# AlexeyAB/yolo2_light

Measured on NVIDIA H100. Metric: images/sec, higher is better.
Workload: dtype bf16

## Files before the change

### yolo2_light_b200/csrc/yb_conv_tc.cu

```cuda
#include <cuda.h>
#include <cuda_bf16.h>
#include <cuda_runtime.h>

#include <algorithm>
#include <climits>
#include <cstdlib>
#include <cstring>
#include <memory>
#include <string>
#include <type_traits>
#include <vector>

#include "yb_conv_tc.cuh"
#include "yb_cuda.h"

namespace yb {

namespace {

constexpr int TC_BM = 128;
constexpr int TC_EPI_WARPS = 8;
constexpr int TC_THREADS = 32 * TC_EPI_WARPS + 32;
constexpr int TC_PRODUCER_WARP = TC_EPI_WARPS;
constexpr int TC_ACC_BAR = 3;
// ... 9 lines not shown
    uint32_t acc;
};

struct TcParams {
    int N;
    int TW, TWlog2, TH;
    int xt, jt, nt;
    int num_work;
    int kind;
    int kk;
    float alpha1;
    const float *mean;
    int xK;
    int *acc_out;
    float *yolo_out;
    int yolo_per;
    int PR, row_off;
    int OH, OW, OHp, OWp;
    int size, cblocks, kblocks;
    int BK, BN;
    int stride2;
    int xoff, yoff;
    int stages;
    uint32_t stage_bytes, a_bytes, b_bytes;
    int bstat;
    uint32_t bstat_bytes;
    int tma_epi;
    uint32_t stg_bytes;
    int acc_pitch;
    int pool_fmt, jshift;
    float pool_mult;
    signed char *pool_out; long pool_ldc; int pool_Hp, pool_Wp;
    int sps;
    TcSmem sm;
    uint32_t desc_hi;
    char *out; long out_ldc; int n;
    const char *res;
    const float *bias; int act, act2;
    unsigned long long *stats;
    int dbg;
};

__device__ __forceinline__ uint32_t smem_u32(const void *p) { return (uint32_t)__cvta_generic_to_shared(p); }

__device__ __forceinline__ bool elect_one() {
    uint32_t pred = 0;
    asm volatile(
        "{\n\t.reg .b32 rx;\n\t.reg .pred px;\n\telect.sync rx|px, %1;\n\t@px mov.s32 %0, 1;\n\t}"
        : "+r"(pred) : "r"(0xffffffffu));
    return pred != 0;
}

__device__ __forceinline__ void mbar_init(uint32_t bar, uint32_t count) {
    asm volatile("mbarrier.init.shared::cta.b64 [%0], %1;" ::"r"(bar), "r"(count));
}
__device__ __forceinline__ void mbar_arrive_expect_tx(uint32_t bar, uint32_t bytes) {
    asm volatile("mbarrier.arrive.expect_tx.shared::cta.b64 _, [%0], %1;" ::"r"(bar), "r"(bytes) : "memory");
}
__device__ __forceinline__ void mbar_arrive(uint32_t bar) {
    asm volatile("mbarrier.arrive.shared::cta.b64 _, [%0];" ::"r"(bar) : "memory");
}
__device__ __forceinline__ uint32_t mbar_try_wait(uint32_t bar, uint32_t parity) {
    uint32_t ok;
    asm volatile(
        "{\n\t.reg .pred p;\n\tmbarrier.try_wait.parity.shared::cta.b64 p, [%1], %2;\n\tselp.b32 %0, 1, 0, p;\n\t}"
        : "=r"(ok) : "r"(bar), "r"(parity) : "memory");
    return ok;
}
__device__ __forceinline__ void mbar_wait(uint32_t bar, uint32_t parity) {
    if (mbar_try_wait(bar, parity)) return;
    const long long t0 = clock64();
    while (!mbar_try_wait(bar, parity))
        if (clock64() - t0 > 4000000000LL) __trap();
}

__device__ __forceinline__ void tma_load_3d(uint32_t dst, const CUtensorMap *tm, uint32_t bar, int c0, int c1, int c2) {
    asm volatile(
        "cp.async.bulk.tensor.3d.shared::cluster.global.tile.mbarrier::complete_tx::bytes [%0], [%1, {%3, %4, %5}], [%2];"
        ::"r"(dst), "l"(tm), "r"(bar), "r"(c0), "r"(c1), "r"(c2) : "memory");
}
__device__ __forceinline__ uint64_t l2_policy_evict_first() {
    uint64_t pol;
    asm volatile("createpolicy.fractional.L2::evict_first.b64 %0, 1.0;" : "=l"(pol));
    return pol;
}
__device__ __forceinline__ void tma_load_3d_hint(uint32_t dst, const CUtensorMap *tm, uint32_t bar, int c0, int c1, int c2, uint64_t pol) {
    asm volatile(
        "cp.async.bulk.tensor.3d.shared::cluster.global.tile.mbarrier::complete_tx::bytes.L2::cache_hint [%0], [%1, {%3, %4, %5}], [%2], %6;"
        ::"r"(dst), "l"(tm), "r"(bar), "r"(c0), "r"(c1), "r"(c2), "l"(pol) : "memory");
}
__device__ __forceinline__ void tma_load_2d(uint32_t dst, const CUtensorMap *tm, uint32_t bar, int c0, int c1) {
    asm volatile(
        "cp.async.bulk.tensor.2d.shared::cluster.global.tile.mbarrier::complete_tx::bytes [%0], [%1, {%3, %4}], [%2];"
        ::"r"(dst), "l"(tm), "r"(bar), "r"(c0), "r"(c1) : "memory");
}
__device__ __forceinline__ void tma_load_5d(uint32_t dst, const CUtensorMap *tm, uint32_t bar, int c0, int c1, int c2,
                                            int c3, int c4) {
    asm volatile(
        "cp.async.bulk.tensor.5d.shared::cluster.global.tile.mbarrier::complete_tx::bytes [%0], [%1, {%3, %4, %5, %6, %7}], [%2];"
        ::"r"(dst), "l"(tm), "r"(bar), "r"(c0), "r"(c1), "r"(c2), "r"(c3), "r"(c4) : "memory");
}

__device__ __forceinline__ void tma_store_3d(const CUtensorMap *tm, uint32_t src, int c0, int c1, int c2) {
    asm volatile("cp.async.bulk.tensor.3d.global.shared::cta.bulk_group [%0, {%2, %3, %4}], [%1];"
                 ::"l"(tm), "r"(src), "r"(c0), "r"(c1), "r"(c2) : "memory");
}
__device__ __forceinline__ void tma_store_commit() { asm volatile("cp.async.bulk.commit_group;" ::: "memory"); }
__device__ __forceinline__ void tma_store_wait_read0() { asm volatile("cp.async.bulk.wait_group.read 0;" ::: "memory"); }
__device__ __forceinline__ void tma_store_wait_all() { asm volatile("cp.async.bulk.wait_group 0;" ::: "memory"); }
__device__ __forceinline__ void named_bar_sync(int id, int nthreads) {
    asm volatile("bar.sync %0, %1;" ::"r"(id), "r"(nthreads) : "memory");
}
__device__ __forceinline__ void prefetch_tmap(const CUtensorMap *tm) { asm volatile("prefetch.tensormap [%0];" ::"l"(tm) : "memory"); }
__device__ __forceinline__ void fence_mbar_init() { asm volatile("fence.mbarrier_init.release.cluster;" ::: "memory"); }
__device__ __forceinline__ void pdl_wait_and_launch() {
    asm volatile("griddepcontrol.wait;" ::: "memory");
    asm volatile("griddepcontrol.launch_dependents;" ::: "memory");
}

__device__ __forceinline__ uint64_t wg_desc(uint32_t addr, uint32_t hi) {
    return ((uint64_t)hi << 32) | (uint64_t)(((addr & 0x3FFFFu) >> 4) | (1u << 16));
}
__device__ __forceinline__ void wg_fence() { asm volatile("wgmma.fence.sync.aligned;" ::: "memory"); }
__device__ __forceinline__ void wg_commit() { asm volatile("wgmma.commit_group.sync.aligned;" ::: "memory"); }
template <int N>
__device__ __forceinline__ void wg_wait() { asm volatile("wgmma.wait_group.sync.aligned %0;" ::"n"(N) : "memory"); }
template <typename T, int N>
// ... 108 lines not shown
};

__device__ __forceinline__ uint32_t pack_bf16x2(float a, float b) {
    __nv_bfloat162 h = __floats2bfloat162_rn(a, b);
    return *reinterpret_cast<uint32_t *>(&h);
}

__device__ __forceinline__ void acc_ld32(uint32_t addr, uint32_t (&v)[32]) {
#pragma unroll
    for (int c = 0; c < 8; ++c)
        asm volatile("ld.shared.v4.b32 {%0, %1, %2, %3}, [%4];" : "=r"(v[4 * c]), "=r"(v[4 * c + 1]), "=r"(v[4 * c + 2]), "=r"(v[4 * c + 3])
                     : "r"(addr + 16u * (uint32_t)c) : "memory");
}
template <typename T, int NR>
__device__ __forceinline__ void acc_store_frag(uint32_t acc, int pitch, int row0, const T (&d)[NR]) {
    const int lane = threadIdx.x & 31, w = (threadIdx.x >> 5) & 3;
    const int r = row0 + 16 * w + (lane >> 2), c = 2 * (lane & 3);
    const uint32_t a0 = acc + 4u * (uint32_t)(r * pitch + c), a1 = a0 + 4u * 8u * (uint32_t)pitch;
#pragma unroll
    for (int j = 0; j < NR / 4; ++j) {
        asm volatile("st.shared.v2.b32 [%0], {%1, %2};" ::"r"(a0 + 32u * (uint32_t)j), "r"(*reinterpret_cast<const uint32_t *>(&d[4 * j])),
                     "r"(*reinterpret_cast<const uint32_t *>(&d[4 * j + 1])) : "memory");
        asm volatile("st.shared.v2.b32 [%0], {%1, %2};" ::"r"(a1 + 32u * (uint32_t)j), "r"(*reinterpret_cast<const uint32_t *>(&d[4 * j + 2])),
                     "r"(*reinterpret_cast<const uint32_t *>(&d[4 * j + 3])) : "memory");
    }
}

__device__ __forceinline__ uint32_t smem_base(const void *smem_raw) { return (smem_u32(smem_raw) + 1023u) & ~1023u; }
__device__ __forceinline__ void *smem_ptr(uint32_t addr) { return __cvta_shared_to_generic(addr); }
__device__ __forceinline__ void st_shared_u32(uint32_t addr, uint32_t v) {
    asm volatile("st.shared.b32 [%0], %1;" ::"r"(addr), "r"(v) : "memory");
}

struct TcItem { int n0, x0, J0; };
__device__ __forceinline__ TcItem tc_item(const TcParams &p, int w, int BN) {
    const int m = w / p.nt;
    return {(w % p.nt) * BN, (m % p.xt) * p.TW, (m / p.xt) * p.TH + p.jshift};
}
struct TcPixel {
    int img, oy, ox;
    __device__ __forceinline__ bool valid(const TcParams &p) const { return img < p.N && oy >= 0 && oy < p.OH && ox < p.OW; }
};
__device__ __forceinline__ TcPixel tc_pixel(const TcParams &p, const TcItem &t, int r) {
    const int J = t.J0 + (r >> p.TWlog2);
    const int img = J / p.PR;
    return {img, J - img * p.PR - p.row_off, t.x0 + (r & (p.TW - 1))};
}

struct TcRing {
    int stage = 0;
    uint32_t phase = 0;
    __device__ __forceinline__ void advance(int stages) { if (++stage == stages) { stage = 0; phase ^= 1u; } }
};
__device__ __forceinline__ void tc_init_ring(const TcParams &p, uint32_t base) {
    for (int s = 0; s < p.stages; ++s) { mbar_init(base + p.sm.full + 8u * s, 1); mbar_init(base + p.sm.empty + 8u * s, TC_EPI_WARPS); }
    mbar_init(base + p.sm.bstat_bar, 1);
}

template <int BN_MAX, typename F>
__device__ __forceinline__ void tc_dispatch(const TcParams &p, F &&f) {
    auto by_kk = [&](auto bn_c) {
        if (p.kk == 4) f(bn_c, std::integral_constant<int, 4>{});
        else if (p.kk == 2) f(bn_c, std::integral_constant<int, 2>{});
        else f(bn_c, std::integral_constant<int, 1>{});
    };
    if constexpr (BN_MAX == 256) {
        if (p.BN == 256) { by_kk(std::integral_constant<int, 256>{}); return; }
    }
    if (p.BN == 128) by_kk(std::integral_constant<int, 128>{});
    else if (p.BN == 64) by_kk(std::integral_constant<int, 64>{});
    else by_kk(std::integral_constant<int, 32>{});
}

enum TcStat {
    STAT_PROD_WAIT_EMPTY,
    STAT_PROD_TMA_ISSUE,
    STAT_PROD_TOTAL,
    STAT_CONS_WAIT_FULL,
    STAT_CONS_WAIT_READY,
    STAT_CONS_FIRST_READY,
    STAT_CONS_TOTAL,
    STAT_STORE_WAIT_FULL,
    STAT_STORE_WAIT_READ,
    TC_NSTATS = 16
};
__device__ __forceinline__ unsigned long long &tc_stat(const TcParams &p, TcStat s) { return p.stats[blockIdx.x * TC_NSTATS + s]; }
template <bool ST, typename F>
__device__ __forceinline__ void timed(long long &cycles, F &&f) {
    if constexpr (ST) { const long long c0 = clock64(); f(); cycles += clock64() - c0; }
    else f();
}

template <bool ST>
__device__ __forceinline__ void tc_produce(const CUtensorMap *tmA, const CUtensorMap *tmB, const TcParams &p, uint32_t base,
                                           int w_first, int w_step) {
    TcRing ring;
    long long w_empty = 0, w_tma = 0; const long long t_begin = ST ? clock64() : 0;
    const int sps = p.sps, kblocks = p.kblocks, cblocks = p.cblocks, BK = p.BK, fsize = p.size, stages = p.stages;
    const int xoff = p.xoff, yoff = p.yoff, stride2 = p.stride2;
    const uint32_t a_bytes = p.a_bytes, b_bytes = p.b_bytes, stage_bytes = p.stage_bytes;
    const uint32_t b_off = (uint32_t)sps * a_bytes;
    const uint32_t smemB = base, smem0 = base + p.sm.ring, bstat_bar = base + p.sm.bstat_bar;
    const int bstat = p.bstat;
    if (bstat) {
        mbar_arrive_expect_tx(bstat_bar, p.bstat_bytes);
        for (int kb = 0; kb < kblocks; ++kb) tma_load_2d(smemB + (uint32_t)kb * b_bytes, tmB, bstat_bar, kb * BK, 0);
    }
    for (int w = w_first; w < p.num_work; w += w_step) {
        const TcItem it = tc_item(p, w, p.BN);
        int cb = 0, ky = 0, kx = 0, kcol = 0;
        for (int kb0 = 0; kb0 < kblocks; kb0 += sps) {
            const int nsub = min(sps, kblocks - kb0);
            timed<ST>(w_empty, [&] { mbar_wait(base + p.sm.empty + 8u * (uint32_t)ring.stage, ring.phase ^ 1u); });
            const uint32_t fb = base + p.sm.full + 8u * (uint32_t)ring.stage;
            const uint32_t a_dst = smem0 + (uint32_t)ring.stage * stage_bytes;
            const uint32_t b_dst = a_dst + b_off;
            if (p.dbg & 1) {
                mbar_arrive(fb);
                ring.advance(stages);
                continue;
            }
            mbar_arrive_expect_tx(fb, (uint32_t)nsub * (a_bytes + (bstat ? 0u : b_bytes)));
            timed<ST>(w_tma, [&] {
                for (int j = 0; j < nsub; ++j) {
                    const uint32_t ad = a_dst + (uint32_t)j * a_bytes, bd = b_dst + (uint32_t)j * b_bytes;
                    const int c0 = cb * BK;
                    if (stride2) tma_load_5d(ad, tmA, fb, c0, kx & 1, it.x0 + (kx >> 1), ky & 1, it.J0 + (ky >> 1));
                    else tma_load_3d(ad, tmA, fb, c0, it.x0 + kx + xoff, it.J0 + ky + yoff);
                    if (!bstat) tma_load_2d(bd, tmB, fb, kcol, it.n0);
                    kcol += BK;
                    if (++cb == cblocks) { cb = 0; if (++kx == fsize) { kx = 0; ++ky; } }
                }
            });
            ring.advance(stages);
        }
    }
    if (ST && p.stats) {
        tc_stat(p, STAT_PROD_WAIT_EMPTY) = w_empty; tc_stat(p, STAT_PROD_TMA_ISSUE) = w_tma;
        tc_stat(p, STAT_PROD_TOTAL) = clock64() - t_begin;
    }
}

template <TcKind KIND, int BN, int KK, bool ST, typename T>
__device__ __forceinline__ void tc_mma_loop(T (&d)[BN / 2], const TcParams &p, uint32_t base, int wg, int lane, TcRing &ring,
                                            long long &w_full) {
#pragma unroll
    for (int i = 0; i < BN / 2; ++i) d[i] = T(0);
    wg_fence_operand(d);
    const int sps = p.sps, stages = p.stages, kblocks = p.kblocks;
    const uint32_t a_bytes = p.a_bytes, b_bytes = p.b_bytes, stage_bytes = p.stage_bytes, hi = p.desc_hi;
    const uint32_t b_off = (uint32_t)sps * a_bytes, a_wg = (uint32_t)wg * (a_bytes >> 1);
    const uint32_t smemB = base, smem0 = base + p.sm.ring;
    const uint32_t full = base + p.sm.full, empty = base + p.sm.empty;
    auto release = [&](int s) { __syncwarp(); if (lane == 0) mbar_arrive(empty + 8u * (uint32_t)s); };
    int pend = -1, jj = 0;
    for (int kb = 0; kb < kblocks; ++kb) {
        if (jj == 0) timed<ST>(w_full, [&] { mbar_wait(full + 8u * (uint32_t)ring.stage, ring.phase); });
        const uint32_t st_base = smem0 + (uint32_t)ring.stage * stage_bytes;
        const uint32_t a_kb = st_base + a_wg + (uint32_t)jj * a_bytes;
        const uint32_t b_kb = p.bstat ? smemB + (uint32_t)kb * b_bytes : st_base + b_off + (uint32_t)jj * b_bytes;
        wg_fence();
#pragma unroll
        for (int k = 0; k < KK; ++k)
            Wg<KIND, BN>::mma(d, wg_desc(a_kb + 32u * (uint32_t)k, hi), wg_desc(b_kb + 32u * (uint32_t)k, hi),
                              (kb > 0 || k > 0) ? 1u : 0u);
        wg_commit();
        wg_wait<1>();
        if (pend >= 0) { release(pend); pend = -1; }
        if (++jj == sps || kb + 1 == kblocks) {
            pend = ring.stage; jj = 0;
            ring.advance(stages);
        }
    }
    wg_wait<0>();
    wg_fence_operand(d);
    if (pend >= 0) release(pend);
}

template <Arith A>
__device__ __forceinline__ float int_epilogue(const TcParams &p, int acc, int f, float bias) {
    return IntEpi<A>::finish(acc, IntEpi<A>::MEAN ? ((f < p.n) ? __ldg(p.mean + f) : 0.f) : p.alpha1, bias, p.act);
}

template <bool ST, int EPI>
__global__ void __launch_bounds__(TC_THREADS, 1)
k_conv_tc(const __grid_constant__ CUtensorMap tmA, const __grid_constant__ CUtensorMap tmB, const __grid_constant__ CUtensorMap tmO,
          const __grid_constant__ CUtensorMap tmO1, const __grid_constant__ CUtensorMap tmR, const TcParams p) {
    extern __shared__ uint8_t smem_raw[];
    const uint32_t base = smem_base(smem_raw);

    const int warp = __shfl_sync(0xffffffffu, (int)(threadIdx.x >> 5), 0);
    const int lane = threadIdx.x & 31;
    const int w_first = (int)blockIdx.x, w_step = (int)gridDim.x;

    if (warp == TC_PRODUCER_WARP && elect_one()) {
        prefetch_tmap(&tmA);
        prefetch_tmap(&tmB);
        tc_init_ring(p, base);
        if (p.tma_epi) prefetch_tmap(&tmO);
        fence_mbar_init();
    }
    const float *bias_s = reinterpret_cast<const float *>(smem_ptr(base + p.sm.bias));
    const uint32_t *ymask_s = reinterpret_cast<const uint32_t *>(smem_ptr(base + p.sm.ymask));
    const uint32_t stg_base = base + p.sm.stg;
    const uint32_t acc_base = base + p.sm.acc;
    for (int i = threadIdx.x; i < p.nt * p.BN; i += TC_THREADS)
        st_shared_u32(base + p.sm.bias + 4u * (uint32_t)i, __float_as_uint((i < p.n) ? __ldg(p.bias + i) : 0.f));
    if (p.yolo_out) {
        for (int wd = threadIdx.x; wd < p.nt * p.BN / 32; wd += TC_THREADS) {
            uint32_t m = 0;
            for (int j = 0; j < 32; ++j) { const int e = (wd * 32 + j) % p.yolo_per; if (e == 2 || e == 3) m |= 1u << j; }
            st_shared_u32(base + p.sm.ymask + 4u * (uint32_t)wd, m);
        }
    }
    __syncthreads();
    pdl_wait_and_launch();

    if (warp == TC_PRODUCER_WARP) {
        if (elect_one()) tc_produce<ST>(&tmA, &tmB, p, base, w_first, w_step);
    } else {
        const int ew = warp;
        const int wg = ew >> 2;
        TcRing ring;
        long long w_full = 0;
        if (p.bstat) mbar_wait(base + p.sm.bstat_bar, 0);
        auto mainloop = [&](auto kind_c) {
            tc_dispatch<128>(p, [&](auto bn_c, auto kk_c) {
                constexpr TcKind KIND = decltype(kind_c)::value;
                constexpr int BN = decltype(bn_c)::value;
                constexpr int KK = decltype(kk_c)::value;
                using T = typename std::conditional<KIND == TC_S8, uint32_t, float>::type;
                T d[BN / 2];
                tc_mma_loop<KIND, BN, KK, ST>(d, p, base, wg, lane, ring, w_full);
                named_bar_sync(TC_ACC_BAR, 32 * TC_EPI_WARPS);
                acc_store_frag(acc_base, p.acc_pitch, wg * 64, d);
                named_bar_sync(TC_ACC_BAR, 32 * TC_EPI_WARPS);
            });
        };
        auto run_mainloop = [&]() {
            if constexpr (EPI == 2) mainloop(std::integral_constant<TcKind, TC_S8>{});
            else if (p.kind == TC_BF16) mainloop(std::integral_constant<TcKind, TC_BF16>{});
            else mainloop(std::integral_constant<TcKind, TC_TF32>{});
        };

        const int q = ew & 3;
        const int half = ew >> 2;
        const int cbeg = (p.BN >= 64) ? half * (p.BN >> 1) : 0;
        const int cend = (p.BN >= 64) ? cbeg + (p.BN >> 1) : (half == 0 ? p.BN : 0);
        const int r = q * 32 + lane;
        const bool leaky = p.act == ACT_LEAKY;
        const uint32_t taddr = acc_base + 4u * (uint32_t)(r * p.acc_pitch);
        const long long t_begin = ST ? clock64() : 0;
// ... 157 lines not shown
                if (p.kind == TC_XNOR) int_slabs(std::integral_constant<Arith, AR_XNOR>{});
                else if (p.kind == TC_S8_GPU) int_slabs(std::integral_constant<Arith, AR_INT8_GPU>{});
                else if (p.kind == TC_XNOR_GPU) int_slabs(std::integral_constant<Arith, AR_XNOR_GPU>{});
                else if (p.kind == TC_PM1Z_GPU) int_slabs(std::integral_constant<Arith, AR_PM1Z_GPU>{});
                else int_slabs(std::integral_constant<Arith, AR_INT8>{});
            } else {
                for (int f0 = cbeg; f0 < cend; f0 += 64) {
                    if (cend - f0 >= 64) {
                        uint32_t v0[32], v1[32];
                        acc_ld32(taddr + 4u * (uint32_t)f0, v0);
                        acc_ld32(taddr + 4u * (uint32_t)f0 + 128u, v1);
                        finish_f32(v0, f0);
                        finish_f32(v1, f0 + 32);
                    } else {
                        uint32_t v0[32];
                        acc_ld32(taddr + 4u * (uint32_t)f0, v0);
                        finish_f32(v0, f0);
                    }
                }
            }
        }
        if (EPI == 2 && p.tma_epi && q == 0 && lane == 0) tma_store_wait_all();
        if (ST && p.stats && ew == 0 && lane == 0) { tc_stat(p, STAT_CONS_WAIT_FULL) = w_full; tc_stat(p, STAT_CONS_TOTAL) = clock64() - t_begin; }
    }
}

constexpr int TCR_THREADS = 384;
constexpr int TCR_PRODUCER_REGS = 40, TCR_CONSUMER_REGS = 216;
constexpr int TCR_STORE_WARP = 9;
constexpr int TCR_MAX_SLABS = 4;

template <bool ST>
__device__ __forceinline__ void tcr_store(const CUtensorMap *tmO, const CUtensorMap *tmO1, const CUtensorMap *tmR, const TcParams &p,
                                          uint32_t buf, uint32_t stg_full, uint32_t stg_ready, int g, int w_first, int w_step) {
    const int SW = p.tma_epi, BN = p.BN;
    const uint32_t tile = 64u * 2u * (uint32_t)SW;
    const int hx = (p.TW == 128) ? 64 * g : 0, hy = (p.TW == 128) ? 0 : g * (p.TH >> 1);
    long long w_full = 0, w_read = 0;
    auto item = [&](int w, int &n0, int &x, int &y) {
        const TcItem it = tc_item(p, w, BN);
        n0 = it.n0; x = it.x0 + 1 + hx; y = it.J0 + hy;
        if (p.stride2) {
            const int i0 = y / p.PR, i1 = min((y + max(p.TH >> 1, 1) - 1) / p.PR, p.N - 1);
            y = i0 == i1 ? y + i0 + 1 : -1 - y;
        }
        return (min(BN, p.n - n0) + SW - 1) / SW;
    };
    auto store_slab = [&](uint32_t src, int c, int x, int y) {
        if (y >= 0) { tma_store_3d(tmO, src, c, x, y); return; }
        const int J0 = -1 - y;
        int img = J0 / p.PR, oy = J0 - img * p.PR;
        for (int t = 0; t < (p.TH >> 1); ++t) {
            if (img < p.N && oy < p.OH) tma_store_3d(tmO1, src, c, x, J0 + t + img + 1);
            if (++oy == p.PR) { oy = 0; ++img; }
            src += (uint32_t)(p.TW * 2 * SW);
        }
    };
    auto wait_read = [&]() { timed<ST>(w_read, tma_store_wait_read0); };
    auto load_res = [&](int s, int n0, int x, int y) {
        tma_load_3d_hint(buf + (uint32_t)s * tile, tmR, stg_ready, n0 + s * SW, x, y, l2_policy_evict_first());
    };
    if (w_first < p.num_work) {
        if (p.res) {
            int n0, x, y;
            const int ns = item(w_first, n0, x, y);
            mbar_arrive_expect_tx(stg_ready, (uint32_t)ns * tile);
            for (int s = 0; s < ns; ++s) load_res(s, n0, x, y);
        } else mbar_arrive(stg_ready);
    }
    uint32_t phases = 0;
    for (int w = w_first; w < p.num_work; w += w_step) {
        int n0, x, y, n0n = 0, xn = 0, yn = 0;
        const int ns = item(w, n0, x, y);
        const bool next = w + w_step < p.num_work, res_next = next && p.res;
        const int nsn = next ? item(w + w_step, n0n, xn, yn) : 0;
        for (int s = 0; s < ns; ++s) {
            const uint32_t fb = stg_full + 8u * (uint32_t)s;
            timed<ST>(w_full, [&] { mbar_wait(fb, (phases >> s) & 1u); });
            phases ^= 1u << s;
            if (s == 0 && res_next) mbar_arrive_expect_tx(stg_ready, (uint32_t)nsn * tile);
            store_slab(buf + (uint32_t)s * tile, n0 + s * SW, x, y);
            tma_store_commit();
            if (res_next && s < nsn) { wait_read(); load_res(s, n0n, xn, yn); }
        }
        if (res_next) {
            for (int s = ns; s < nsn; ++s) { wait_read(); load_res(s, n0n, xn, yn); }
        } else if (next) {
            wait_read();
            mbar_arrive(stg_ready);
        }
    }
    tma_store_wait_all();
    if (ST && p.stats && g == 0) { tc_stat(p, STAT_STORE_WAIT_FULL) = w_full; tc_stat(p, STAT_STORE_WAIT_READ) = w_read; }
}

template <bool ST>
__global__ void __launch_bounds__(TCR_THREADS, 1)
k_conv_tc_reg(const __grid_constant__ CUtensorMap tmA, const __grid_constant__ CUtensorMap tmB, const __grid_constant__ CUtensorMap tmO,
              const __grid_constant__ CUtensorMap tmO1, const __grid_constant__ CUtensorMap tmR, const TcParams p) {
    extern __shared__ uint8_t smem_raw[];
    const uint32_t base = smem_base(smem_raw);
    auto stg_full = [&](int g, int s) { return base + p.sm.stg_full + 8u * (uint32_t)(g * TCR_MAX_SLABS + s); };
    auto stg_ready = [&](int g) { return base + p.sm.stg_ready + 8u * (uint32_t)g; };
    float *bias_s = reinterpret_cast<float *>(smem_ptr(base + p.sm.bias));
    const uint32_t stg_base = base + p.sm.stg;

    const int warp = __shfl_sync(0xffffffffu, (int)(threadIdx.x >> 5), 0);
    const int lane = threadIdx.x & 31;
    const int wg = warp >> 2;
    const int w_first = (int)blockIdx.x, w_step = (int)gridDim.x;
    const bool epi_mem = !(p.dbg & 4);

    if (warp == TC_PRODUCER_WARP && elect_one()) {
        prefetch_tmap(&tmA);
        prefetch_tmap(&tmB);
        prefetch_tmap(&tmO);
        if (p.stride2) prefetch_tmap(&tmO1);
        if (p.res) prefetch_tmap(&tmR);
        tc_init_ring(p, base);
        for (int g = 0; g < 2; ++g) {
            for (int s = 0; s < TCR_MAX_SLABS; ++s) mbar_init(stg_full(g, s), 4);
            mbar_init(stg_ready(g), 1);
        }
        fence_mbar_init();
    }
    for (int i = threadIdx.x; i < p.nt * p.BN; i += TCR_THREADS) bias_s[i] = (i < p.n) ? __ldg(p.bias + i) : 0.f;
    __syncthreads();
    pdl_wait_and_launch();

    if (wg == 2) {
        asm volatile("setmaxnreg.dec.sync.aligned.u32 %0;" ::"n"(TCR_PRODUCER_REGS));
        if (warp == TC_PRODUCER_WARP) {
            if (elect_one()) tc_produce<ST>(&tmA, &tmB, p, base, w_first, w_step);
        } else if (warp < TCR_STORE_WARP + 2 && epi_mem) {
            const int g = warp - TCR_STORE_WARP;
            if (elect_one()) tcr_store<ST>(&tmO, &tmO1, &tmR, p, stg_base + (uint32_t)g * 128u * (uint32_t)p.BN, stg_full(g, 0), stg_ready(g), g, w_first, w_step);
        }
        return;
    }
    asm volatile("setmaxnreg.inc.sync.aligned.u32 %0;" ::"n"(TCR_CONSUMER_REGS));

    const int rl = 16 * (warp & 3) + (lane >> 2), cq = 2 * (lane & 3);
    const bool leaky = p.act == ACT_LEAKY, leaky2 = p.act2 == ACT_LEAKY;
    const bool has_res = p.res != nullptr;
    TcRing ring;
    uint32_t stg_phase = 0;
    long long w_full = 0, w_ready = 0; const long long t_begin = ST ? clock64() : 0;
    if (p.bstat) mbar_wait(base + p.sm.bstat_bar, 0);

    tc_dispatch<256>(p, [&](auto bn_c, auto kk_c) {
        constexpr int BN = decltype(bn_c)::value;
        constexpr int KK = decltype(kk_c)::value;
        constexpr int SW = BN >= 64 ? 64 : 32;
        constexpr uint32_t ROWB = SW * 2, TILE = 64u * ROWB;
        const uint32_t buf = stg_base + (uint32_t)wg * (uint32_t)(BN / SW) * TILE;
        auto slab_off = [&](int row, int c) -> uint32_t {
            const int sw = (SW == 64) ? (row & 7) : ((row >> 1) & 3);
            return (uint32_t)row * ROWB + ((uint32_t)(c ^ sw) << 4) + 2u * (uint32_t)cq;
        };
        for (int w = w_first; w < p.num_work; w += w_step) {
            float d[BN / 2];
            tc_mma_loop<TC_BF16, BN, KK, ST>(d, p, base, wg, lane, ring, w_full);
            if (!epi_mem) continue;
            const TcItem it = tc_item(p, w, BN);
            const int n0 = it.n0;
            bool valid[2];
#pragma unroll
            for (int h = 0; h < 2; ++h)
                valid[h] = tc_pixel(p, it, 64 * wg + rl + 8 * h).valid(p);
            const int nslab = (min(BN, p.n - n0) + SW - 1) / SW;
            long long dt = 0;
            timed<ST>(dt, [&] { mbar_wait(stg_ready(wg), stg_phase); });
            if (w != w_first) w_ready += dt;
            else if (ST && p.stats && warp == 0 && lane == 0) tc_stat(p, STAT_CONS_FIRST_READY) = dt;
            stg_phase ^= 1u;
#pragma unroll
            for (int s = 0; s < BN / SW; ++s) {
                if (s >= nslab) break;
                const uint32_t slab = buf + (uint32_t)s * TILE;
#pragma unroll
                for (int jj = 0; jj < SW / 8; ++jj) {
                    const int j = s * (SW / 8) + jj;
                    const float2 b = *reinterpret_cast<const float2 *>(bias_s + n0 + 8 * j + cq);
#pragma unroll
                    for (int e = 0; e < 4; ++e) {
                        const float a = d[4 * j + e] + ((e & 1) ? b.y : b.x);
                        d[4 * j + e] = leaky ? fmaxf(a, 0.1f * a) : a;
                    }
                }
                if (has_res) {
                    uint32_t u[SW / 8][2];
#pragma unroll
                    for (int jj = 0; jj < SW / 8; ++jj)
#pragma unroll
                        for (int h = 0; h < 2; ++h)
                            asm volatile("ld.shared.b32 %0, [%1];" : "=r"(u[jj][h]) : "r"(slab + slab_off(rl + 8 * h, jj)));
#pragma unroll
                    for (int jj = 0; jj < SW / 8; ++jj) {
                        const int j = s * (SW / 8) + jj;
#pragma unroll
                        for (int h = 0; h < 2; ++h) {
                            float a = d[4 * j + 2 * h] + __uint_as_float(u[jj][h] << 16);
                            float c = d[4 * j + 2 * h + 1] + __uint_as_float(u[jj][h] & 0xffff0000u);
                            if (leaky2) { a = fmaxf(a, 0.1f * a); c = fmaxf(c, 0.1f * c); }
                            d[4 * j + 2 * h] = a; d[4 * j + 2 * h + 1] = c;
                        }
                    }
                }
#pragma unroll
                for (int jj = 0; jj < SW / 8; ++jj) {
                    const int j = s * (SW / 8) + jj;
#pragma unroll
                    for (int h = 0; h < 2; ++h) {
                        const uint32_t o = valid[h] ? pack_bf16x2(d[4 * j + 2 * h], d[4 * j + 2 * h + 1]) : 0u;
                        asm volatile("st.shared.b32 [%0], %1;" ::"r"(slab + slab_off(rl + 8 * h, jj)), "r"(o));
                    }
                }
                asm volatile("fence.proxy.async.shared::cta;" ::: "memory");
                __syncwarp();
                if (lane == 0) mbar_arrive(stg_full(wg, s));
            }
        }
    });
    if (ST && p.stats && warp == 0 && lane == 0) {
        tc_stat(p, STAT_CONS_WAIT_FULL) = w_full; tc_stat(p, STAT_CONS_WAIT_READY) = w_ready;
        tc_stat(p, STAT_CONS_TOTAL) = clock64() - t_begin;
    }
}

struct StemTcP {
    const float *in;
    const unsigned char *in8;
    char *out; int out_ldc;
    const __nv_bfloat16 *w;
    const float *bias;
    int N, H, W, OHp, OWp, nf, act;
    long npix;
    int ntiles;
    const __nv_bfloat16 *w1;
    const float *bias1;
    int act1, OH, OW, xt, yt;
};

template <bool U8>
__global__ void __launch_bounds__(128) k_stem_tc(StemTcP p) {
    __shared__ __align__(1024) uint8_t a_tile[128 * 64];
    __shared__ __align__(1024) uint8_t b_tile[32 * 64];
    __shared__ __align__(16) float acc_s[128 * 36];
    __shared__ float bias_s[32];
    __shared__ unsigned long long optr[128];
    __shared__ float lut[U8 ? 256 : 1];
    const int t = threadIdx.x;
    if constexpr (U8) { lut[t] = (float)((double)(float)t / 255.0); lut[t + 128] = (float)((double)(float)(t + 128) / 255.0); }
    const uint32_t a_addr = smem_u32(a_tile), b_addr = smem_u32(b_tile), acc_addr = smem_u32(acc_s);
    if (t < 32) bias_s[t] = (t < p.nf) ? p.bias[t] : 0.f;
    {
        const int f = t >> 2, j = t & 3;
        const uint4 v = *reinterpret_cast<const uint4 *>(p.w + f * 32 + j * 8);
        *reinterpret_cast<uint4 *>(b_tile + f * 64 + ((j ^ ((f >> 1) & 3)) << 4)) = v;
    }
// ... 526 lines not shown
}

void encode_maps(TcPlan &plan, const TcConv &c, bool reg) {
    const TcParams &p = plan.p;
    const TV &in = c.in;
    const int esz = elem_size(c.kind), cin = operand_channels(c);
    const CUtensorMapSwizzle swz = p.kk == 4 ? CU_TENSOR_MAP_SWIZZLE_128B : p.kk == 2 ? CU_TENSOR_MAP_SWIZZLE_64B : CU_TENSOR_MAP_SWIZZLE_32B;
    const CUtensorMapDataType dtype = c.kind == TC_TF32 ? CU_TENSOR_MAP_DATA_TYPE_FLOAT32
                                    : is_integer(c.kind) ? CU_TENSOR_MAP_DATA_TYPE_UINT8 : CU_TENSOR_MAP_DATA_TYPE_BFLOAT16;
    EncodeTiledFn enc = encode_fn();
    auto check = [](CUresult r, const char *what) {
        if (r != CUDA_SUCCESS) fatal_throw(std::string("cuTensorMapEncodeTiled(") + what + ") failed: " + std::to_string((int)r));
    };
    if (!p.stride2) {
        cuuint64_t dims[3] = {(cuuint64_t)cin, (cuuint64_t)in.Wp, (cuuint64_t)in.N * in.Hp};
        cuuint64_t strides[2] = {(cuuint64_t)in.ldc * esz, (cuuint64_t)in.Wp * in.ldc * esz};
        cuuint32_t box[3] = {(cuuint32_t)p.BK, (cuuint32_t)p.TW, (cuuint32_t)p.TH};
        cuuint32_t es[3] = {1, 1, 1};
        check(enc(&plan.tmA, dtype, 3, in.base, dims, strides, box, es,
                  CU_TENSOR_MAP_INTERLEAVE_NONE, swz, CU_TENSOR_MAP_L2_PROMOTION_L2_128B, CU_TENSOR_MAP_FLOAT_OOB_FILL_NONE), "A");
    } else {
        cuuint64_t dims[5] = {(cuuint64_t)cin, 2, (cuuint64_t)in.Wp / 2, 2, (cuuint64_t)in.N * in.Hp / 2};
        cuuint64_t strides[4] = {(cuuint64_t)in.ldc * esz, (cuuint64_t)in.ldc * 2 * esz, (cuuint64_t)in.Wp * in.ldc * esz,
                                 (cuuint64_t)in.Wp * in.ldc * 2 * esz};
        cuuint32_t box[5] = {(cuuint32_t)p.BK, 1, (cuuint32_t)p.TW, 1, (cuuint32_t)p.TH};
        cuuint32_t es[5] = {1, 1, 1, 1, 1};
        check(enc(&plan.tmA, dtype, 5, in.base, dims, strides, box, es,
                  CU_TENSOR_MAP_INTERLEAVE_NONE, swz, CU_TENSOR_MAP_L2_PROMOTION_L2_128B, CU_TENSOR_MAP_FLOAT_OOB_FILL_NONE), "A");
    }
    {
        const cuuint64_t K = (cuuint64_t)p.size * p.size * cin;
        cuuint64_t dims[2] = {K, (cuuint64_t)c.ldn};
        cuuint64_t strides[1] = {K * esz};
        cuuint32_t box[2] = {(cuuint32_t)p.BK, (cuuint32_t)p.BN};
        cuuint32_t es[2] = {1, 1};
        check(enc(&plan.tmB, dtype, 2, const_cast<void *>(c.w), dims, strides, box, es,
                  CU_TENSOR_MAP_INTERLEAVE_NONE, swz, CU_TENSOR_MAP_L2_PROMOTION_L2_256B, CU_TENSOR_MAP_FLOAT_OOB_FILL_NONE), "B");
    }
    plan.tmO = plan.tmA; plan.tmO1 = plan.tmA; plan.tmR = plan.tmA;
    if (p.tma_epi && c.out.base) {
        const int oesz = c.out_bf16 ? 2 : 4;
        auto encode_px = [&](CUtensorMap *tm, const TV &t, const char *what, int box_rows) {
            cuuint64_t dims[3] = {(cuuint64_t)p.n, (cuuint64_t)t.Wp, (cuuint64_t)t.N * t.Hp};
            cuuint64_t strides[2] = {(cuuint64_t)t.ldc * oesz, (cuuint64_t)t.Wp * t.ldc * oesz};
            cuuint32_t box[3] = {(cuuint32_t)p.tma_epi, (cuuint32_t)std::min(p.TW, reg ? 64 : 128), (cuuint32_t)box_rows};
            cuuint32_t es[3] = {1, 1, 1};
            check(enc(tm, c.out_bf16 ? CU_TENSOR_MAP_DATA_TYPE_BFLOAT16 : CU_TENSOR_MAP_DATA_TYPE_FLOAT32, 3, t.base, dims, strides, box, es,
                      CU_TENSOR_MAP_INTERLEAVE_NONE, p.tma_epi * oesz == 128 ? CU_TENSOR_MAP_SWIZZLE_128B : CU_TENSOR_MAP_SWIZZLE_64B,
                      CU_TENSOR_MAP_L2_PROMOTION_L2_128B, CU_TENSOR_MAP_FLOAT_OOB_FILL_NONE), what);
        };
        const int box_rows = reg ? std::max(p.TH / 2, 1) : p.TH;
        encode_px(&plan.tmO, c.out, "output", box_rows);
        if (reg && p.stride2) encode_px(&plan.tmO1, c.out, "output row", 1);
        if (c.res.base) encode_px(&plan.tmR, c.res, "residual", box_rows);
    }
}

}

int tc_conv_supported(const TcConv &c) {
    const Layer &l = *c.l;
    const bool integer = is_integer(c.kind);
    auto aligned = [](const TV &t, int esz) { return (reinterpret_cast<uintptr_t>(t.base) & 15) == 0 && t.ldc * esz % 16 == 0; };
    if (!geometry_ok(l) || l.n < 8 || (l.activation != YB_LEAKY && l.activation != YB_LINEAR)) return 0;
    if (channel_row(operand_channels(c), elem_size(c.kind)) == 0 || c.in.P != 1 || !aligned(c.in, elem_size(c.kind))) return 0;
    if (c.out_bf16 && (c.kind != TC_BF16 || l.n % 8 != 0)) return 0;
    if (c.out.base ? (c.out.P != 1 || !aligned(c.out, c.out_bf16 ? 2 : 4)) : !(c.yolo_out || c.pool_fmt != SIDE_NONE)) return 0;
    if (c.res.base && !(c.kind == TC_BF16 && c.out_bf16 && l.stride == 1 && c.res.H == l.out_h && c.res.W == l.out_w &&
                        c.res.C == l.n && aligned(c.res, 2)))
        return 0;
    if (c.yolo_out && (integer || c.out_bf16)) return 0;
    if (c.pool_fmt != SIDE_NONE && !(integer && (side_s8(c.pool_fmt) || c.pool_fmt == SIDE_PM1_S8) && !c.acc_out && l.size == 3 && l.stride == 1 &&
                         l.h % 2 == 0 && l.out_h % 2 == 0 && l.out_w % 2 == 0 && l.n % 32 == 0 &&
                         c.pool_next.H == l.out_h / 2 && c.pool_next.W == l.out_w / 2 && aligned(c.pool_next, 1)))
        return 0;
    return 1;
}

TcPlanPtr tc_make_plan(const TcConv &c) {
    const Layer &l = *c.l;
    if (!tc_conv_supported(c)) fatal_throw("tc plan: convolution not supported by the tensor-core kernels");
    TcPlanPtr plan(new TcPlan());
    TcParams &p = plan->p;
    const bool reg = c.kind == TC_BF16 && c.out_bf16;
    const int sms = sm_count();
    plan_tiles(p, c, reg, sms);
    plan_epilogue(p, c, reg);
    plan_ring(p, reg);
    plan->smem = tc_smem_layout(p, reg);
    p.dbg = c.sw.dbg;
    snprintf(plan->desc, sizeof(plan->desc), "%dx%dx%d -> n%d k%d s%d%s", l.c, l.h, l.w, l.n, l.size, l.stride, reg ? " reg" : "");
    encode_maps(*plan, c, reg);
    plan->grid = std::min(p.num_work, grid_cap(sms, c.sw.grid));
    const bool st = c.sw.stats;
    plan->reg = reg;
    if (reg) plan->kernel = st ? k_conv_tc_reg<true> : k_conv_tc_reg<false>;
    else if (is_integer(c.kind)) plan->kernel = st ? k_conv_tc<true, 2> : k_conv_tc<false, 2>;
    else plan->kernel = st ? k_conv_tc<true, 0> : k_conv_tc<false, 0>;
    if (cudaFuncSetAttribute((const void *)plan->kernel, cudaFuncAttributeMaxDynamicSharedMemorySize, 227 * 1024) != cudaSuccess)
        fatal_throw("cudaFuncSetAttribute(k_conv_tc) failed");
    if (st) {
        plan->stats.ensure(TC_NSTATS * (size_t)plan->grid);
        p.stats = plan->stats.get();
        cudaMemset(p.stats, 0, sizeof(unsigned long long) * TC_NSTATS * plan->grid);
    }
    return plan;
}

struct StemPlan { StemTcP p; int grid; bool s2; };
int tc_stem_supported(const Layer &l, const TV &out) {
    return l.c == 3 && l.size == 3 && l.stride == 1 && l.pad == 1 && (l.n == 16 || l.n == 32) &&
           (l.activation == YB_LEAKY || l.activation == YB_LINEAR) && out.base && out.ldc % 8 == 0 &&
           (reinterpret_cast<uintptr_t>(out.base) & 15) == 0;
}
StemPlanPtr tc_stem_make_plan(const Layer &l, const TV &out, const void *d_w, const float *d_bias) {
    StemPlanPtr sp(new StemPlan());
    StemTcP &p = sp->p;
    p.out = out.base; p.out_ldc = out.ldc; p.w = reinterpret_cast<const __nv_bfloat16 *>(d_w); p.bias = d_bias;
    p.N = out.N; p.H = l.h; p.W = l.w; p.OHp = out.Hp; p.OWp = out.Wp; p.nf = l.n; p.act = l.activation;
    p.npix = (long)out.N * l.h * l.w;
    if (p.npix >= (1L << 31) - 256) fatal_throw("stem plan: more than 2^31 pixels per batch");
    p.ntiles = (int)((p.npix + 127) / 128);
    sp->grid = std::min(p.ntiles, sm_count() * 8);
    return sp;
}
int tc_stem_s2_supported(const Layer &l0, const Layer &l1, const TV &out1) {
    return l0.n == 32 && l1.c == 32 && l1.n == 64 && l1.size == 3 && l1.stride == 2 && l1.pad == 1 && l1.h == l0.h && l1.w == l0.w &&
           l0.h % 2 == 0 && l0.w % 2 == 0 && (l1.activation == YB_LEAKY || l1.activation == YB_LINEAR) && out1.base && out1.P == 1 &&
           out1.H == l0.h / 2 && out1.W == l0.w / 2 && out1.ldc % 8 == 0 && (reinterpret_cast<uintptr_t>(out1.base) & 15) == 0;
}
StemPlanPtr tc_stem_s2_make_plan(const Layer &l0, const Layer &l1, const TV &out1, const void *d_w, const float *d_bias,
                                 const void *d_w1, const float *d_bias1, int max_grid) {
    StemPlanPtr sp(new StemPlan());
// ... 21 lines not shown
    if (sp.s2) k_stem_s2_tc<false><<<sp.grid, 256, S2_SMEM, s>>>(p);
    else k_stem_tc<false><<<sp.grid, 128, 0, s>>>(p);
}
void tc_stem_launch_u8(const StemPlan &sp, const unsigned char *d_in_hwc, cudaStream_t s) {
    StemTcP p = sp.p;
    p.in8 = d_in_hwc;
    if (sp.s2) k_stem_s2_tc<true><<<sp.grid, 256, S2_SMEM, s>>>(p);
    else k_stem_tc<true><<<sp.grid, 128, 0, s>>>(p);
}

namespace {
int copy_fields(const int (&f)[TC_PLAN_NFIELDS], int *fields, int n) {
    const int k = std::max(0, std::min(n, (int)TC_PLAN_NFIELDS));
    for (int i = 0; i < k; ++i) fields[i] = f[i];
    return k;
}
}

int tc_plan_fields(const TcPlan &plan, int *fields, int n) {
    const TcParams &p = plan.p;
    const int f[TC_PLAN_NFIELDS] = {plan.reg ? TC_PLAN_CONV_REG : TC_PLAN_CONV, p.kind, p.TW, p.TH, p.BN, p.BK,
                                    p.nt, p.bstat, p.stages, p.sps, plan.grid, p.num_work, p.tma_epi, p.jshift,
                                    p.out ? (int)p.out_ldc : 0};
    return copy_fields(f, fields, n);
}

int tc_stem_plan_fields(const StemPlan &sp, int *fields, int n) {
    const int f[TC_PLAN_NFIELDS] = {sp.s2 ? TC_PLAN_STEM_S2 : TC_PLAN_STEM, TC_BF16, sp.s2 ? S2_TW : -1, sp.s2 ? S2_TH : -1,
                                    sp.s2 ? 64 : -1, -1, -1, -1, -1, -1, sp.grid, sp.p.ntiles, -1, -1, (int)sp.p.out_ldc};
    return copy_fields(f, fields, n);
}

void tc_launch(const TcPlan &P, cudaStream_t s) {
    cudaLaunchConfig_t cfg{};
    cfg.gridDim = dim3((unsigned)P.grid); cfg.blockDim = dim3((unsigned)(P.reg ? TCR_THREADS : TC_THREADS));
    cfg.dynamicSmemBytes = P.smem; cfg.stream = s;
    cudaLaunchAttribute attr[1];
    attr[0].id = cudaLaunchAttributeProgrammaticStreamSerialization;
    attr[0].val.programmaticStreamSerializationAllowed = 1;
    cfg.attrs = attr; cfg.numAttrs = 1;
    cudaLaunchKernelEx(&cfg, P.kernel, P.tmA, P.tmB, P.tmO, P.tmO1, P.tmR, P.p);
}

void TcPlanDelete::operator()(TcPlan *plan) const {
    if (plan->p.stats) {
        std::vector<unsigned long long> h(TC_NSTATS * (size_t)plan->grid);
        cudaDeviceSynchronize();
        cudaMemcpy(h.data(), plan->p.stats, h.size() * sizeof(unsigned long long), cudaMemcpyDeviceToHost);
        double m[TC_NSTATS] = {0};
        for (int b = 0; b < plan->grid; ++b) for (int k = 0; k < TC_NSTATS; ++k) m[k] += (double)h[TC_NSTATS * b + k] / plan->grid;
        fprintf(stderr, "TCSTATS %-28s tiles/cta %.1f kb %d sps %d BN %d | producer: wait_empty %.0f tma_issue %.0f total %.0f | ",
                plan->desc, (double)plan->p.num_work / plan->grid, plan->p.kblocks, plan->p.sps, plan->p.BN,
                m[STAT_PROD_WAIT_EMPTY], m[STAT_PROD_TMA_ISSUE], m[STAT_PROD_TOTAL]);
        if (plan->reg)
            fprintf(stderr, "consumers: wait_full %.0f wait_ready %.0f (first item %.0f) total %.0f | store: wait_full %.0f wait_read %.0f\n",
                    m[STAT_CONS_WAIT_FULL], m[STAT_CONS_WAIT_READY], m[STAT_CONS_FIRST_READY], m[STAT_CONS_TOTAL],
                    m[STAT_STORE_WAIT_FULL], m[STAT_STORE_WAIT_READ]);
        else fprintf(stderr, "consumers: wait_full %.0f total %.0f\n", m[STAT_CONS_WAIT_FULL], m[STAT_CONS_TOTAL]);
    }
    delete plan;
}
void TcPlanDelete::operator()(StemPlan *plan) const { delete plan; }

}
```

Measured before the change: 3174.

## Multicast weight tiles across 2-CTA clusters for BN=256 register-epilogue convs

Pairs adjacent CTAs into 2-CTA clusters that work on neighbouring M tiles sharing the same N tile. Each CTA TMA-loads half of the B (weight) tile and multicasts it to both CTAs. Empty barriers now count arrivals from both CTAs, and the work schedule is remapped so paired CTAs stay in lockstep. The aim is to halve global/L2 weight traffic per CTA, at the cost of cross-CTA synchronization coupling, cluster launch constraints, and a solo path for an odd final tile.

New measurement: 2988 (median of 6 runs). 5.9% lower.

```diff
diff --git a/yolo2_light_b200/csrc/yb_conv_tc.cu b/yolo2_light_b200/csrc/yb_conv_tc.cu
--- a/yolo2_light_b200/csrc/yb_conv_tc.cu
+++ b/yolo2_light_b200/csrc/yb_conv_tc.cu
@@ -65,6 +65,7 @@
     float pool_mult;
     signed char *pool_out; long pool_ldc; int pool_Hp, pool_Wp;
     int sps;
+    int pair;
     TcSmem sm;
     uint32_t desc_hi;
     char *out; long out_ldc; int n;
@@ -93,6 +94,20 @@
 __device__ __forceinline__ void mbar_arrive(uint32_t bar) {
     asm volatile("mbarrier.arrive.shared::cta.b64 _, [%0];" ::"r"(bar) : "memory");
 }
+__device__ __forceinline__ void mbar_arrive2(uint32_t bar) {
+    asm volatile("mbarrier.arrive.shared::cta.b64 _, [%0], 2;" ::"r"(bar) : "memory");
+}
+__device__ __forceinline__ void mbar_arrive_cluster(uint32_t cbar) {
+    asm volatile("mbarrier.arrive.shared::cluster.b64 _, [%0];" ::"r"(cbar) : "memory");
+}
+__device__ __forceinline__ uint32_t mapa_peer(uint32_t addr) {
+    uint32_t r;
+    asm volatile("mapa.shared::cluster.u32 %0, %1, %2;" : "=r"(r) : "r"(addr), "r"((blockIdx.x & 1u) ^ 1u));
+    return r;
+}
+__device__ __forceinline__ void cluster_sync() {
+    asm volatile("barrier.cluster.arrive.release;\n\tbarrier.cluster.wait.acquire;" ::: "memory");
+}
 __device__ __forceinline__ uint32_t mbar_try_wait(uint32_t bar, uint32_t parity) {
     uint32_t ok;
     asm volatile(
@@ -126,6 +141,11 @@
     asm volatile(
         "cp.async.bulk.tensor.2d.shared::cluster.global.tile.mbarrier::complete_tx::bytes [%0], [%1, {%3, %4}], [%2];"
         ::"r"(dst), "l"(tm), "r"(bar), "r"(c0), "r"(c1) : "memory");
+}
+__device__ __forceinline__ void tma_load_2d_pair(uint32_t dst, const CUtensorMap *tm, uint32_t bar, int c0, int c1) {
+    asm volatile(
+        "cp.async.bulk.tensor.2d.shared::cluster.global.tile.mbarrier::complete_tx::bytes.multicast::cluster [%0], [%1, {%3, %4}], [%2], %5;"
+        ::"r"(dst), "l"(tm), "r"(bar), "r"(c0), "r"(c1), "h"((uint16_t)0x3) : "memory");
 }
 __device__ __forceinline__ void tma_load_5d(uint32_t dst, const CUtensorMap *tm, uint32_t bar, int c0, int c1, int c2,
                                             int c3, int c4) {
@@ -300,6 +320,19 @@
     asm volatile("st.shared.b32 [%0], %1;" ::"r"(addr), "r"(v) : "memory");
 }
 
+__device__ __forceinline__ int tc_work(const TcParams &p, int k) {
+    if (!p.pair) {
+        const int w = (int)blockIdx.x + k * (int)gridDim.x;
+        return w < p.num_work ? w : -1;
+    }
+    const int q = (int)(blockIdx.x >> 1) + k * (int)(gridDim.x >> 1);
+    const int mp = q / p.nt, m = 2 * mp + (int)(blockIdx.x & 1);
+    return m < p.xt * p.jt ? m * p.nt + (q - mp * p.nt) : -1;
+}
+__device__ __forceinline__ bool tc_solo(const TcParams &p, int w) {
+    const int M = p.xt * p.jt;
+    return p.pair && (M & 1) && w / p.nt == M - 1;
+}
 struct TcItem { int n0, x0, J0; };
 __device__ __forceinline__ TcItem tc_item(const TcParams &p, int w, int BN) {
     const int m = w / p.nt;
@@ -321,7 +354,10 @@
     __device__ __forceinline__ void advance(int stages) { if (++stage == stages) { stage = 0; phase ^= 1u; } }
 };
 __device__ __forceinline__ void tc_init_ring(const TcParams &p, uint32_t base) {
-    for (int s = 0; s < p.stages; ++s) { mbar_init(base + p.sm.full + 8u * s, 1); mbar_init(base + p.sm.empty + 8u * s, TC_EPI_WARPS); }
+    for (int s = 0; s < p.stages; ++s) {
+        mbar_init(base + p.sm.full + 8u * s, 1);
+        mbar_init(base + p.sm.empty + 8u * s, p.pair ? 2 * TC_EPI_WARPS : TC_EPI_WARPS);
+    }
     mbar_init(base + p.sm.bstat_bar, 1);
 }
 
@@ -360,8 +396,7 @@
 }
 
 template <bool ST>
-__device__ __forceinline__ void tc_produce(const CUtensorMap *tmA, const CUtensorMap *tmB, const TcParams &p, uint32_t base,
-                                           int w_first, int w_step) {
+__device__ __forceinline__ void tc_produce(const CUtensorMap *tmA, const CUtensorMap *tmB, const TcParams &p, uint32_t base) {
     TcRing ring;
     long long w_empty = 0, w_tma = 0; const long long t_begin = ST ? clock64() : 0;
     const int sps = p.sps, kblocks = p.kblocks, cblocks = p.cblocks, BK = p.BK, fsize = p.size, stages = p.stages;
@@ -374,8 +409,10 @@
         mbar_arrive_expect_tx(bstat_bar, p.bstat_bytes);
         for (int kb = 0; kb < kblocks; ++kb) tma_load_2d(smemB + (uint32_t)kb * b_bytes, tmB, bstat_bar, kb * BK, 0);
     }
-    for (int w = w_first; w < p.num_work; w += w_step) {
+    int w;
+    for (int k = 0; (w = tc_work(p, k)) >= 0; ++k) {
         const TcItem it = tc_item(p, w, p.BN);
+        const bool solo = tc_solo(p, w);
         int cb = 0, ky = 0, kx = 0, kcol = 0;
         for (int kb0 = 0; kb0 < kblocks; kb0 += sps) {
             const int nsub = min(sps, kblocks - kb0);
@@ -395,7 +432,15 @@
                     const int c0 = cb * BK;
                     if (stride2) tma_load_5d(ad, tmA, fb, c0, kx & 1, it.x0 + (kx >> 1), ky & 1, it.J0 + (ky >> 1));
                     else tma_load_3d(ad, tmA, fb, c0, it.x0 + kx + xoff, it.J0 + ky + yoff);
-                    if (!bstat) tma_load_2d(bd, tmB, fb, kcol, it.n0);
+                    if (!p.pair) {
+                        if (!bstat) tma_load_2d(bd, tmB, fb, kcol, it.n0);
+                    } else if (!solo) {
+                        const int rank = (int)(blockIdx.x & 1);
+                        tma_load_2d_pair(bd + (uint32_t)rank * (b_bytes >> 1), tmB, fb, kcol, it.n0 + rank * (p.BN >> 1));
+                    } else {
+                        tma_load_2d(bd, tmB, fb, kcol, it.n0);
+                        tma_load_2d(bd + (b_bytes >> 1), tmB, fb, kcol, it.n0 + (p.BN >> 1));
+                    }
                     kcol += BK;
                     if (++cb == cblocks) { cb = 0; if (++kx == fsize) { kx = 0; ++ky; } }
                 }
@@ -411,7 +456,7 @@
 
 template <TcKind KIND, int BN, int KK, bool ST, typename T>
 __device__ __forceinline__ void tc_mma_loop(T (&d)[BN / 2], const TcParams &p, uint32_t base, int wg, int lane, TcRing &ring,
-                                            long long &w_full) {
+                                            long long &w_full, bool solo = false) {
 #pragma unroll
     for (int i = 0; i < BN / 2; ++i) d[i] = T(0);
     wg_fence_operand(d);
@@ -420,7 +465,14 @@
     const uint32_t b_off = (uint32_t)sps * a_bytes, a_wg = (uint32_t)wg * (a_bytes >> 1);
     const uint32_t smemB = base, smem0 = base + p.sm.ring;
     const uint32_t full = base + p.sm.full, empty = base + p.sm.empty;
-    auto release = [&](int s) { __syncwarp(); if (lane == 0) mbar_arrive(empty + 8u * (uint32_t)s); };
+    auto release = [&](int s) {
+        __syncwarp();
+        if (lane != 0) return;
+        const uint32_t e = empty + 8u * (uint32_t)s;
+        if (!p.pair) mbar_arrive(e);
+        else if (solo) mbar_arrive2(e);
+        else { mbar_arrive(e); mbar_arrive_cluster(mapa_peer(e)); }
+    };
     int pend = -1, jj = 0;
     for (int kb = 0; kb < kblocks; ++kb) {
         if (jj == 0) timed<ST>(w_full, [&] { mbar_wait(full + 8u * (uint32_t)ring.stage, ring.phase); });
@@ -485,7 +537,7 @@
     pdl_wait_and_launch();
 
     if (warp == TC_PRODUCER_WARP) {
-        if (elect_one()) tc_produce<ST>(&tmA, &tmB, p, base, w_first, w_step);
+        if (elect_one()) tc_produce<ST>(&tmA, &tmB, p, base);
     } else {
         const int ew = warp;
         const int wg = ew >> 2;
@@ -709,7 +761,7 @@
 
 template <bool ST>
 __device__ __forceinline__ void tcr_store(const CUtensorMap *tmO, const CUtensorMap *tmO1, const CUtensorMap *tmR, const TcParams &p,
-                                          uint32_t buf, uint32_t stg_full, uint32_t stg_ready, int g, int w_first, int w_step) {
+                                          uint32_t buf, uint32_t stg_full, uint32_t stg_ready, int g) {
     const int SW = p.tma_epi, BN = p.BN;
     const uint32_t tile = 64u * 2u * (uint32_t)SW;
     const int hx = (p.TW == 128) ? 64 * g : 0, hy = (p.TW == 128) ? 0 : g * (p.TH >> 1);
@@ -737,20 +789,22 @@
     auto load_res = [&](int s, int n0, int x, int y) {
         tma_load_3d_hint(buf + (uint32_t)s * tile, tmR, stg_ready, n0 + s * SW, x, y, l2_policy_evict_first());
     };
-    if (w_first < p.num_work) {
+    int w = tc_work(p, 0);
+    if (w >= 0) {
         if (p.res) {
             int n0, x, y;
-            const int ns = item(w_first, n0, x, y);
+            const int ns = item(w, n0, x, y);
             mbar_arrive_expect_tx(stg_ready, (uint32_t)ns * tile);
             for (int s = 0; s < ns; ++s) load_res(s, n0, x, y);
         } else mbar_arrive(stg_ready);
     }
     uint32_t phases = 0;
-    for (int w = w_first; w < p.num_work; w += w_step) {
+    for (int k = 0; w >= 0; ++k) {
         int n0, x, y, n0n = 0, xn = 0, yn = 0;
         const int ns = item(w, n0, x, y);
-        const bool next = w + w_step < p.num_work, res_next = next && p.res;
-        const int nsn = next ? item(w + w_step, n0n, xn, yn) : 0;
+        const int wn = tc_work(p, k + 1);
+        const bool next = wn >= 0, res_next = next && p.res;
+        const int nsn = next ? item(wn, n0n, xn, yn) : 0;
         for (int s = 0; s < ns; ++s) {
             const uint32_t fb = stg_full + 8u * (uint32_t)s;
             timed<ST>(w_full, [&] { mbar_wait(fb, (phases >> s) & 1u); });
@@ -766,6 +820,7 @@
             wait_read();
             mbar_arrive(stg_ready);
         }
+        w = wn;
     }
     tma_store_wait_all();
     if (ST && p.stats && g == 0) { tc_stat(p, STAT_STORE_WAIT_FULL) = w_full; tc_stat(p, STAT_STORE_WAIT_READ) = w_read; }
@@ -785,7 +840,6 @@
     const int warp = __shfl_sync(0xffffffffu, (int)(threadIdx.x >> 5), 0);
     const int lane = threadIdx.x & 31;
     const int wg = warp >> 2;
-    const int w_first = (int)blockIdx.x, w_step = (int)gridDim.x;
     const bool epi_mem = !(p.dbg & 4);
 
     if (warp == TC_PRODUCER_WARP && elect_one()) {
@@ -803,16 +857,18 @@
     }
     for (int i = threadIdx.x; i < p.nt * p.BN; i += TCR_THREADS) bias_s[i] = (i < p.n) ? __ldg(p.bias + i) : 0.f;
     __syncthreads();
+    if (p.pair) cluster_sync();
     pdl_wait_and_launch();
 
     if (wg == 2) {
         asm volatile("setmaxnreg.dec.sync.aligned.u32 %0;" ::"n"(TCR_PRODUCER_REGS));
         if (warp == TC_PRODUCER_WARP) {
-            if (elect_one()) tc_produce<ST>(&tmA, &tmB, p, base, w_first, w_step);
+            if (elect_one()) tc_produce<ST>(&tmA, &tmB, p, base);
         } else if (warp < TCR_STORE_WARP + 2 && epi_mem) {
             const int g = warp - TCR_STORE_WARP;
-            if (elect_one()) tcr_store<ST>(&tmO, &tmO1, &tmR, p, stg_base + (uint32_t)g * 128u * (uint32_t)p.BN, stg_full(g, 0), stg_ready(g), g, w_first, w_step);
-        }
+            if (elect_one()) tcr_store<ST>(&tmO, &tmO1, &tmR, p, stg_base + (uint32_t)g * 128u * (uint32_t)p.BN, stg_full(g, 0), stg_ready(g), g);
+        }
+        if (p.pair) cluster_sync();
         return;
     }
     asm volatile("setmaxnreg.inc.sync.aligned.u32 %0;" ::"n"(TCR_CONSUMER_REGS));
@@ -835,9 +891,10 @@
             const int sw = (SW == 64) ? (row & 7) : ((row >> 1) & 3);
             return (uint32_t)row * ROWB + ((uint32_t)(c ^ sw) << 4) + 2u * (uint32_t)cq;
         };
-        for (int w = w_first; w < p.num_work; w += w_step) {
+        int w;
+        for (int k = 0; (w = tc_work(p, k)) >= 0; ++k) {
             float d[BN / 2];
-            tc_mma_loop<TC_BF16, BN, KK, ST>(d, p, base, wg, lane, ring, w_full);
+            tc_mma_loop<TC_BF16, BN, KK, ST>(d, p, base, wg, lane, ring, w_full, tc_solo(p, w));
             if (!epi_mem) continue;
             const TcItem it = tc_item(p, w, BN);
             const int n0 = it.n0;
@@ -848,7 +905,7 @@
             const int nslab = (min(BN, p.n - n0) + SW - 1) / SW;
             long long dt = 0;
             timed<ST>(dt, [&] { mbar_wait(stg_ready(wg), stg_phase); });
-            if (w != w_first) w_ready += dt;
+            if (k != 0) w_ready += dt;
             else if (ST && p.stats && warp == 0 && lane == 0) tc_stat(p, STAT_CONS_FIRST_READY) = dt;
             stg_phase ^= 1u;
 #pragma unroll
@@ -903,6 +960,7 @@
         tc_stat(p, STAT_CONS_WAIT_FULL) = w_full; tc_stat(p, STAT_CONS_WAIT_READY) = w_ready;
         tc_stat(p, STAT_CONS_TOTAL) = clock64() - t_begin;
     }
+    if (p.pair) cluster_sync();
 }
 
 struct StemTcP {
@@ -1495,7 +1553,7 @@
         const cuuint64_t K = (cuuint64_t)p.size * p.size * cin;
         cuuint64_t dims[2] = {K, (cuuint64_t)c.ldn};
         cuuint64_t strides[1] = {K * esz};
-        cuuint32_t box[2] = {(cuuint32_t)p.BK, (cuuint32_t)p.BN};
+        cuuint32_t box[2] = {(cuuint32_t)p.BK, (cuuint32_t)(p.pair ? p.BN / 2 : p.BN)};
         cuuint32_t es[2] = {1, 1};
         check(enc(&plan.tmB, dtype, 2, const_cast<void *>(c.w), dims, strides, box, es,
                   CU_TENSOR_MAP_INTERLEAVE_NONE, swz, CU_TENSOR_MAP_L2_PROMOTION_L2_256B, CU_TENSOR_MAP_FLOAT_OOB_FILL_NONE), "B");
@@ -1517,6 +1575,27 @@
         if (reg && p.stride2) encode_px(&plan.tmO1, c.out, "output row", 1);
         if (c.res.base) encode_px(&plan.tmR, c.res, "residual", box_rows);
     }
+}
+
+cudaLaunchConfig_t launch_config(const TcPlan &P) {
+    cudaLaunchConfig_t cfg{};
+    cfg.gridDim = dim3((unsigned)P.grid); cfg.blockDim = dim3((unsigned)(P.reg ? TCR_THREADS : TC_THREADS));
+    cfg.dynamicSmemBytes = P.smem;
+    return cfg;
+}
+cudaLaunchAttribute pair_attr() {
+    cudaLaunchAttribute a{};
+    a.id = cudaLaunchAttributeClusterDimension;
+    a.val.clusterDim.x = 2; a.val.clusterDim.y = 1; a.val.clusterDim.z = 1;
+    return a;
+}
+int pair_clusters(const TcPlan &P) {
+    cudaLaunchConfig_t cfg = launch_config(P);
+    cudaLaunchAttribute a = pair_attr();
+    cfg.attrs = &a; cfg.numAttrs = 1;
+    int n = 0;
+    if (cudaOccupancyMaxActiveClusters(&n, (const void *)P.kernel, &cfg) != cudaSuccess) { cudaGetLastError(); return 0; }
+    return n;
 }
 
 }
@@ -1553,7 +1632,6 @@
     plan->smem = tc_smem_layout(p, reg);
     p.dbg = c.sw.dbg;
     snprintf(plan->desc, sizeof(plan->desc), "%dx%dx%d -> n%d k%d s%d%s", l.c, l.h, l.w, l.n, l.size, l.stride, reg ? " reg" : "");
-    encode_maps(*plan, c, reg);
     plan->grid = std::min(p.num_work, grid_cap(sms, c.sw.grid));
     const bool st = c.sw.stats;
     plan->reg = reg;
@@ -1562,6 +1640,8 @@
     else plan->kernel = st ? k_conv_tc<true, 0> : k_conv_tc<false, 0>;
     if (cudaFuncSetAttribute((const void *)plan->kernel, cudaFuncAttributeMaxDynamicSharedMemorySize, 227 * 1024) != cudaSuccess)
         fatal_throw("cudaFuncSetAttribute(k_conv_tc) failed");
+    p.pair = reg && !p.bstat && p.BN == 256 && plan->grid % 2 == 0 && pair_clusters(*plan) >= plan->grid / 2;
+    encode_maps(*plan, c, reg);
     if (st) {
         plan->stats.ensure(TC_NSTATS * (size_t)plan->grid);
         p.stats = plan->stats.get();
@@ -1649,13 +1729,13 @@
 }
 
 void tc_launch(const TcPlan &P, cudaStream_t s) {
-    cudaLaunchConfig_t cfg{};
-    cfg.gridDim = dim3((unsigned)P.grid); cfg.blockDim = dim3((unsigned)(P.reg ? TCR_THREADS : TC_THREADS));
-    cfg.dynamicSmemBytes = P.smem; cfg.stream = s;
-    cudaLaunchAttribute attr[1];
+    cudaLaunchConfig_t cfg = launch_config(P);
+    cfg.stream = s;
+    cudaLaunchAttribute attr[2];
     attr[0].id = cudaLaunchAttributeProgrammaticStreamSerialization;
     attr[0].val.programmaticStreamSerializationAllowed = 1;
-    cfg.attrs = attr; cfg.numAttrs = 1;
+    attr[1] = pair_attr();
+    cfg.attrs = attr; cfg.numAttrs = P.p.pair ? 2 : 1;
     cudaLaunchKernelEx(&cfg, P.kernel, P.tmA, P.tmB, P.tmO, P.tmO1, P.tmR, P.p);
 }
 
```
